# tiantianxuabc/ORB_SLAM2_Refactored

Measured on AMD Instinct MI355X. Metric: frames/sec ORB extract+match (1280×720, 8 lvl, 1000 feat) + LocalBA iters/sec, higher is better.
Workload: dtype u8; 1 GPU; C2: 1280x720 mono, 8 levels, 2000 features, extract + brute-force Hamming top-2/ratio match of every frame vs its predecessor; width=1280, height=720, nlevels=8, nfeatures=2000, parallelism=8192-frame job sharded over 1 GPU(s), 8192 frames per GPU

## Files before the change

orb_slam2_refactored_amd/csrc/orbx.hip:

```cpp
#include <algorithm>
#include <cfloat>
#include <cmath>
#include <cstring>
#include <mutex>
#include <type_traits>
#include <vector>

#include <hip/hip_ext.h>

#include "common.h"
#include "qt_sort.h"
#include "sincos_f.h"
#include "stereo.h"

namespace orbamd {

constexpr int MAX_LEVELS = 16;
constexpr int MAX_ZONE = 64;
constexpr int MAX_ROOTS = 32;
constexpr int PATCH = 43;
constexpr int HBLUR_W = 37;
constexpr int HBS = 40;
static_assert(HBLUR_W + 3 <= HBS, "the blur's fourth-column tiles store up to column 39");

// ... 116 lines not shown
}

template <bool WV>
__device__ __forceinline__ void qt_sync() {
    if constexpr (WV) {
        __builtin_amdgcn_fence(__ATOMIC_ACQ_REL, "workgroup");
        __builtin_amdgcn_wave_barrier();
        asm volatile("s_waitcnt lgkmcnt(0)" ::: "memory");
    } else {
        __syncthreads();
    }
}
template <bool WV>
__device__ __forceinline__ int grp_excl_scan(int v, int* tmp, int* total) {
    if constexpr (WV) {
        const int inc = wave_incl_scan(v);
        *total = __builtin_amdgcn_readlane(inc, 63);
        return inc - v;
    } else {
        return block_excl_scan(v, tmp, total);
    }
}

typedef unsigned short us2 __attribute__((ext_vector_type(2)));

__device__ __forceinline__ uint32_t htap24(uint32_t h) { return h & 0xffff0u; }
__device__ __forceinline__ uint32_t mulhi24(uint32_t a, uint32_t b) {
#ifdef PYR_MULHI_MASK_DIAG
    return __umulhi(a & 0xffffffu, b & 0xffffffu);
#else
    uint32_t r;
    asm("v_mul_hi_u32_u24 %0, %1, %2" : "=v"(r) : "v"(a), "v"(b));
    return r;
#endif
}
__device__ __forceinline__ uint32_t vcoef24(int b) { return ((uint32_t)b & 0xfffu) << 12; }
__device__ __forceinline__ uint32_t vtail(uint32_t h0, uint32_t h1, uint32_t b0_24, uint32_t b1_24) {
    return (__umul24(h0, b0_24 >> 12) + __umul24(h1, b1_24 >> 12) + (1u << 21)) >> 22;
}

__device__ __forceinline__ us2 pyr_tap(uint32_t hi, uint32_t lo, uint32_t sel) {
    const uint32_t r = __builtin_amdgcn_perm(hi, lo, sel);
    return *reinterpret_cast<const us2*>(&r);
}

constexpr int PYR_TW = 64, PYR_TH = 64;
constexpr int PYR_SW = 144, PYR_SH = 128;

__device__ __forceinline__ int4 pyr_row_taps(int2 yv, int sy_lo) {
    return make_int4(((yv.x & 0xffff) - sy_lo) * PYR_SW, ((yv.x >> 16) - sy_lo) * PYR_SW, (int)vcoef24(yv.y),
                     (int)vcoef24(yv.y >> 16));
}

__device__ __forceinline__ void pyr_tile_compute(const Geom& g, const LevelDev& L, int f, uint8_t* pyr,
                                                 const uint8_t* S, const int2* xs_t, const int4* ys_t, int tx0,
                                                 int ty0, int tw, int th, int xa) {
    {
        const int q0 = (threadIdx.x & 15) * 4;
        uint32_t sel0[2], sel1[2];
        int wdb[2];
        us2 a0[2], a1[2];
        bool fits = true;
#pragma unroll
        for (int j = 0; j < 2; j++) {
            const int2 xv0 = xs_t[min(q0 + 2 * j, tw - 1)], xv1 = xs_t[min(q0 + 2 * j + 1, tw - 1)];
            const int s00 = (xv0.x & 0xffff) - xa, s01 = (xv0.x >> 16) - xa;
            const int s10 = (xv1.x & 0xffff) - xa, s11 = (xv1.x >> 16) - xa;
            const int wd = s00 >> 2;
            const int e00 = s00 - 4 * wd, e01 = s01 - 4 * wd, e10 = s10 - 4 * wd, e11 = s11 - 4 * wd;
            fits = fits && max(e01, e11) <= 7 && min(e00, e10) >= 0;
            sel0[j] = (uint32_t)e00 | 0x0c00u | ((uint32_t)e01 << 16) | 0x0c000000u;
            sel1[j] = (uint32_t)e10 | 0x0c00u | ((uint32_t)e11 << 16) | 0x0c000000u;
            wdb[j] = 4 * wd;
            a0[j] = *reinterpret_cast<const us2*>(&xv0.y);
            a1[j] = *reinterpret_cast<const us2*>(&xv1.y);
        }
        if (!__syncthreads_or(!fits)) {
            if (q0 >= tw) return;
            const bool full = q0 + 3 < tw;
            uint8_t* dst = pyr + (long long)f * g.pyr_frame_bytes + L.off + tx0 + q0 +
                           (long long)(ty0 + (int)(threadIdx.x >> 4)) * L.stride;
            const long long dstep = 16ll * L.stride;
            const int tcol = L.tail_x - (tx0 + q0);
            auto rows = [&](auto tail_c) {
                constexpr bool TAIL = decltype(tail_c)::value;
                for (int ty = threadIdx.x >> 4; ty < th; ty += 16, dst += dstep) {
                    const int4 yv = ys_t[ty];
                    const uint32_t b0 = (uint32_t)yv.z, b1 = (uint32_t)yv.w;
                    uint32_t out = 0;
#pragma unroll
                    for (int j = 0; j < 2; j++) {
                        const uint32_t* s0 = reinterpret_cast<const uint32_t*>(S + yv.x + wdb[j]);
                        const uint32_t* s1 = reinterpret_cast<const uint32_t*>(S + yv.y + wdb[j]);
                        const uint32_t w00 = s0[0], w01 = s0[1], w10 = s1[0], w11 = s1[1];
                        const uint32_t r0a = __builtin_amdgcn_udot2(pyr_tap(w01, w00, sel0[j]), a0[j], 0u, false);
                        const uint32_t r1a = __builtin_amdgcn_udot2(pyr_tap(w11, w10, sel0[j]), a0[j], 0u, false);
                        const uint32_t r0b = __builtin_amdgcn_udot2(pyr_tap(w01, w00, sel1[j]), a1[j], 0u, false);
                        const uint32_t r1b = __builtin_amdgcn_udot2(pyr_tap(w11, w10, sel1[j]), a1[j], 0u, false);
                        uint32_t va = (mulhi24(htap24(r0a), b0) + mulhi24(htap24(r1a), b1) + 2) >> 2;
                        uint32_t vb = (mulhi24(htap24(r0b), b0) + mulhi24(htap24(r1b), b1) + 2) >> 2;
                        if (TAIL) {
                            va = 2 * j >= tcol ? vtail(r0a, r1a, b0, b1) : va;
                            vb = 2 * j + 1 >= tcol ? vtail(r0b, r1b, b0, b1) : vb;
                        }
                        out |= (va | (vb << 8)) << (16 * j);
                    }
                    if (full) {
                        *reinterpret_cast<uint32_t*>(dst) = out;
                    } else {
                        for (int k = 0; k < 3; k++)
                            if (q0 + k < tw) dst[k] = (uint8_t)(out >> (8 * k));
                    }
                }
            };
#ifndef PYR_NO_TAIL_DIAG
            if (tx0 + tw > L.tail_x) rows(std::true_type{});
            else
#endif
                rows(std::false_type{});
            return;
        }
    }
    const int q0 = (threadIdx.x & 15) * 4;
    if (q0 >= tw) return;
    uint8_t* dbase = pyr + (long long)f * g.pyr_frame_bytes + L.off + tx0 + q0;
#pragma nounroll
    for (int ty = threadIdx.x >> 4; ty < th; ty += 16) {
        const int4 yv = ys_t[ty];
        const int r0 = yv.x, r1 = yv.y;
        const int b0 = yv.z >> 12, b1 = yv.w >> 12;
        uint32_t packed = 0;
#pragma nounroll
        for (int k = 0; k < 4; k++) {
            const int2 xv = xs_t[min(q0 + k, tw - 1)];
            const int sx0 = (xv.x & 0xffff) - xa, sx1 = (xv.x >> 16) - xa, a0 = xv.y & 0xffff, a1 = xv.y >> 16;
            const int h0 = S[r0 + sx0] * a0 + S[r0 + sx1] * a1;
            const int h1 = S[r1 + sx0] * a0 + S[r1 + sx1] * a1;
            const int s0 = min(h0 >> 4, 32767), s1 = min(h1 >> 4, 32767);
            int v = (((s0 * b0) >> 16) + ((s1 * b1) >> 16) + 2) >> 2;
            if (tx0 + q0 + k >= L.tail_x) v = (h0 * b0 + h1 * b1 + (1 << 21)) >> 22;
            packed |= (uint32_t)(v > 255 ? 255 : v) << (8 * k);
        }
        uint8_t* dst = dbase + (long long)(ty0 + ty) * L.stride;
        if (q0 + 3 < tw) *reinterpret_cast<uint32_t*>(dst) = packed;
        else {
            dst[0] = (uint8_t)packed;
            if (q0 + 1 < tw) dst[1] = (uint8_t)(packed >> 8);
            if (q0 + 2 < tw) dst[2] = (uint8_t)(packed >> 16);
        }
    }
}

constexpr int PYR_PF = 5;

struct PyrTile {
    int f, tx0, ty0, tw, th, sy_lo, xa, nc, items, mul;
    const uint8_t* src;
    int sstep;
};

__device__ __forceinline__ PyrTile pyr_tile_geom(const Geom& g, int l, int t, int ntx, int nty, const uint8_t* in,
                                                 long long in_fstride, int in_step, uint8_t* pyr) {
    const LevelDev& L = g.lv[l];
    const LevelDev& Ls = g.lv[l - 1];
    PyrTile T;
    const int per = ntx * nty;
    T.f = t / per;
    const int r = t - T.f * per;
    T.ty0 = (r / ntx) * PYR_TH;
    T.tx0 = (r - (r / ntx) * ntx) * PYR_TW;
    T.tw = min(PYR_TW, L.w - T.tx0);
    T.th = min(PYR_TH, L.h - T.ty0);
    const int sx_lo = max(0, (int)floor((T.tx0 + 0.5) * L.ssx - 0.5) - 2);
    const int sx_hi = min(Ls.w - 1, (int)floor((T.tx0 + T.tw - 0.5) * L.ssx - 0.5) + 2);
    T.sy_lo = max(0, (int)floor((T.ty0 + 0.5) * L.ssy - 0.5) - 2);
    const int sy_hi = min(Ls.h - 1, (int)floor((T.ty0 + T.th - 0.5) * L.ssy - 0.5) + 2);
    T.xa = sx_lo & ~15;
    T.nc = ((sx_hi - T.xa) >> 4) + 1;
    T.items = (sy_hi - T.sy_lo + 1) * T.nc;
    T.mul = ((1 << 20) + T.nc - 1) / T.nc;
    T.src = level_base(g, l - 1, T.f, in, in_fstride, in_step, pyr, &T.sstep);
    auto u = [](int x) { return __builtin_amdgcn_readfirstlane(x); };
    T.f = u(T.f), T.tx0 = u(T.tx0), T.ty0 = u(T.ty0), T.tw = u(T.tw), T.th = u(T.th), T.sy_lo = u(T.sy_lo);
    T.xa = u(T.xa), T.nc = u(T.nc), T.items = u(T.items), T.mul = u(T.mul), T.sstep = u(T.sstep);
    const unsigned long long sp = (unsigned long long)(uintptr_t)T.src;
    T.src = (const uint8_t*)(uintptr_t)(((unsigned long long)(unsigned)u((int)(sp >> 32)) << 32) |
                                        (unsigned)u((int)(unsigned)sp));
    return T;
}

__device__ __forceinline__ int pyr_piece_row(const PyrTile& T, int i) {
    return (int)(__umulhi(((unsigned)i & 0x7ffu) << 12, (unsigned)T.mul & 0xffffffu) & 0x7ffu);
}
__device__ __forceinline__ int mul12(int a, int b) {
    return (int)(((unsigned)a & 0xfffu) * ((unsigned)b & 0xfffu));
}
__device__ __forceinline__ void pyr_piece_load(const PyrTile& T, int i, uint4& v) {
    if (i < T.items) {
        const int rr = pyr_piece_row(T, i), c = i - mul12(rr, T.nc);
        v = *reinterpret_cast<const uint4*>(T.src + __mul24(T.sy_lo + rr, T.sstep) + T.xa + 16 * c);
    }
}

__device__ __forceinline__ void pyr_fetch(const PyrTile& T, int tid, uint4& v0, uint4& v1, uint4& v2, uint4& v3,
                                          uint4& v4) {
    static_assert(PYR_PF == 5, "five pieces per thread");
    pyr_piece_load(T, tid, v0);
    pyr_piece_load(T, tid + 256, v1);
    pyr_piece_load(T, tid + 512, v2);
    pyr_piece_load(T, tid + 768, v3);
    pyr_piece_load(T, tid + 1024, v4);
}

__device__ __forceinline__ void pyr_stage(const PyrTile& T, int tid, uint8_t* S, const uint4& v, int k) {
    const int i = tid + 256 * k;
    if (i < T.items) {
        const int rr = pyr_piece_row(T, i), c = i - mul12(rr, T.nc);
        *reinterpret_cast<uint4*>(&S[mul12(rr, PYR_SW) + 16 * c]) = v;
    }
}

__global__ __launch_bounds__(256) void pyramid_level_kernel(Geom g, int l, const uint8_t* __restrict__ in,
                                                            long long in_fstride, int in_step, uint8_t* pyr,
                                                            const int2* __restrict__ xtab,
                                                            const int2* __restrict__ ytab) {
    __shared__ __attribute__((aligned(16))) uint8_t S[PYR_SH * PYR_SW + 16];
    __shared__ int2 xs_t[PYR_TW];
    __shared__ int4 ys_t[PYR_TH];
    const LevelDev& L = g.lv[l];
    const LevelDev& Ls = g.lv[l - 1];
    const int gx = gridDim.x, gxy = gridDim.x * gridDim.y;
    const int lb = xcd_swizzle(blockIdx.x + gx * blockIdx.y + gxy * blockIdx.z, gxy * gridDim.z);
    const int f = lb / gxy;
    const int tx0 = (lb % gx) * PYR_TW, ty0 = ((lb % gxy) / gx) * PYR_TH;
    const int tw = min(PYR_TW, L.w - tx0), th = min(PYR_TH, L.h - ty0);
    int sstep;
    const uint8_t* src = level_base(g, l - 1, f, in, in_fstride, in_step, pyr, &sstep);
    const int2* xt = xtab + L.xtab_off;
    const int2* yt = ytab + L.ytab_off;
    const int sw = Ls.w, sh = Ls.h;
    const double scx = L.ssx, scy = L.ssy;
    const int sx_lo = max(0, (int)floor((tx0 + 0.5) * scx - 0.5) - 2);
    const int sx_hi = min(sw - 1, (int)floor((tx0 + tw - 0.5) * scx - 0.5) + 2);
    const int sy_lo = max(0, (int)floor((ty0 + 0.5) * scy - 0.5) - 2);
    if ((int)threadIdx.x < tw) xs_t[threadIdx.x] = xt[tx0 + threadIdx.x];
    if ((int)threadIdx.x >= 64 && (int)threadIdx.x - 64 < th)
        ys_t[threadIdx.x - 64] = pyr_row_taps(yt[ty0 + threadIdx.x - 64], sy_lo);
    const int sy_hi = min(sh - 1, (int)floor((ty0 + th - 0.5) * scy - 0.5) + 2);
    const int xa = sx_lo & ~3;
    const int nd = (sx_hi - xa + 4) >> 2;
    const int nr = sy_hi - sy_lo + 1;
    const bool aligned = ((reinterpret_cast<uintptr_t>(src) | (uintptr_t)sstep) & 3) == 0;
    if (((reinterpret_cast<uintptr_t>(src) | (uintptr_t)sstep) & 15) == 0 && sx_hi - (sx_lo & ~15) < PYR_SW) {
        const PyrTile T = pyr_tile_geom(g, l, lb, gx, gridDim.y, in, in_fstride, in_step, pyr);
        uint4 v0, v1, v2, v3, v4;
        pyr_fetch(T, threadIdx.x, v0, v1, v2, v3, v4);
        pyr_stage(T, threadIdx.x, S, v0, 0);
        pyr_stage(T, threadIdx.x, S, v1, 1);
        pyr_stage(T, threadIdx.x, S, v2, 2);
        pyr_stage(T, threadIdx.x, S, v3, 3);
        pyr_stage(T, threadIdx.x, S, v4, 4);
        __syncthreads();
        pyr_tile_compute(g, L, f, pyr, S, xs_t, ys_t, tx0, ty0, tw, th, T.xa);
        return;
    }
    if (aligned) {
        constexpr int RPW = PYR_SH / 4;
        const int wv = __builtin_amdgcn_readfirstlane((int)(threadIdx.x >> 6));
        const int ln = threadIdx.x & 63;
        const int col = min(xa + 4 * ln, (sw - 1) & ~3);
        const uint8_t* rbase = src + (long long)sy_lo * sstep + col;
        uint32_t v[RPW];
#pragma unroll
        for (int k = 0; k < RPW; k++) {
            const int rk = min(wv + 4 * k, nr - 1);
            v[k] = *reinterpret_cast<const uint32_t*>(rbase + (long long)rk * sstep);
        }
        if (ln < nd) {
            uint32_t* drow = reinterpret_cast<uint32_t*>(S) + wv * (PYR_SW / 4) + ln;
#pragma unroll
            for (int k = 0; k < RPW; k++)
                if (wv + 4 * k < nr) drow[k * PYR_SW] = v[k];
        }
    } else {
        for (int i = threadIdx.x; i < nd * nr; i += blockDim.x) {
            const int r = i / nd, d = i - r * nd;
            const uint8_t* rowp = src + (long long)(sy_lo + r) * sstep;
            const int x = xa + 4 * d;
            uint32_t v = 0;
            for (int q = 0; q < 4; q++)
                if (x + q < sw) v |= (uint32_t)rowp[x + q] << (8 * q);
            *reinterpret_cast<uint32_t*>(&S[r * PYR_SW + 4 * d]) = v;
        }
    }
    __syncthreads();
    pyr_tile_compute(g, L, f, pyr, S, xs_t, ys_t, tx0, ty0, tw, th, xa);
}

constexpr int PP_MAXP = 8;
constexpr int PP_MAXC = 96, PP_MAXR = 96;

__device__ __forceinline__ uint32_t pyr_px_generic(const uint8_t* S, int2 xv, int4 yv, int xa, bool tail) {
    const int r0 = yv.x, r1 = yv.y;
    const int sx0 = (xv.x & 0xffff) - xa, sx1 = (xv.x >> 16) - xa, a0 = xv.y & 0xffff, a1 = xv.y >> 16;
    const int b0 = yv.z >> 12, b1 = yv.w >> 12;
    const int h0 = S[r0 + sx0] * a0 + S[r0 + sx1] * a1;
    const int h1 = S[r1 + sx0] * a0 + S[r1 + sx1] * a1;
    const int s0 = min(h0 >> 4, 32767), s1 = min(h1 >> 4, 32767);
    int v = (((s0 * b0) >> 16) + ((s1 * b1) >> 16) + 2) >> 2;
    if (tail) v = (h0 * b0 + h1 * b1 + (1 << 21)) >> 22;
    return (uint32_t)(v > 255 ? 255 : v);
}

__global__ __launch_bounds__(256) void pyramid_pair_kernel(Geom g, int l, const uint8_t* __restrict__ in,
                                                           long long in_fstride, int in_step, uint8_t* pyr,
                                                           const int2* __restrict__ xtab,
                                                           const int2* __restrict__ ytab) {
    __shared__ __attribute__((aligned(16))) uint8_t S[PYR_SH * PYR_SW + 16];
    __shared__ int2 xs1[PP_MAXC], xs2[PYR_TW];
    __shared__ int4 ys1[PP_MAXR], ys2[PYR_TH];
    const LevelDev& L0 = g.lv[l - 1];
    const LevelDev& L1 = g.lv[l];
    const LevelDev& L2 = g.lv[l + 1];
    const int tid = threadIdx.x;
    const int gx = gridDim.x, gxy = gridDim.x * gridDim.y;
    const int lb = xcd_swizzle(blockIdx.x + gx * blockIdx.y + gxy * blockIdx.z, gxy * gridDim.z);
    const int f = lb / gxy;
    const int tx0 = (lb % gx) * PYR_TW, ty0 = ((lb % gxy) / gx) * PYR_TH;
    const int tw = min(PYR_TW, L2.w - tx0), th = min(PYR_TH, L2.h - ty0);
    auto u = [](int x) { return __builtin_amdgcn_readfirstlane(x); };
    const int ax0 = max(0, (int)floor((tx0 + 0.5) * L2.ssx - 0.5) - 2);
    const int c1 = u(min(L1.w - 1, (int)floor((tx0 + tw - 0.5) * L2.ssx - 0.5) + 2));
    const int ay0 = u(max(0, (int)floor((ty0 + 0.5) * L2.ssy - 0.5) - 2));
    const int ay1 = u(min(L1.h - 1, (int)floor((ty0 + th - 0.5) * L2.ssy - 0.5) + 2));
    const int c0 = u(ax0 & ~3);
    const int ncol = c1 - c0 + 1, nrow = ay1 - ay0 + 1;
    PyrTile T;
    const int bx0 = max(0, (int)floor((c0 + 0.5) * L1.ssx - 0.5) - 2);
    const int bx1 = min(L0.w - 1, (int)floor((c1 + 0.5) * L1.ssx - 0.5) + 2);
    T.sy_lo = u(max(0, (int)floor((ay0 + 0.5) * L1.ssy - 0.5) - 2));
    const int by1 = min(L0.h - 1, (int)floor((ay1 + 0.5) * L1.ssy - 0.5) + 2);
    T.xa = u(bx0 & ~15);
    T.nc = u(((bx1 - T.xa) >> 4) + 1);
    T.items = u((by1 - T.sy_lo + 1) * T.nc);
    T.mul = u(((1 << 20) + T.nc - 1) / T.nc);
    T.src = level_base(g, l - 1, f, in, in_fstride, in_step, pyr, &T.sstep);
    {
        uint4 v0, v1, v2, v3, v4;
        pyr_fetch(T, tid, v0, v1, v2, v3, v4);
        if (tid < ncol) xs1[tid] = xtab[L1.xtab_off + c0 + tid];
// ... 53 lines not shown
                        const uint32_t r0b = __builtin_amdgcn_udot2(pyr_tap(w01, w00, sel1[j]), a1[j], 0u, false);
                        const uint32_t r1b = __builtin_amdgcn_udot2(pyr_tap(w11, w10, sel1[j]), a1[j], 0u, false);
                        uint32_t va = (mulhi24(htap24(r0a), b0) + mulhi24(htap24(r1a), b1) + 2) >> 2;
                        uint32_t vb = (mulhi24(htap24(r0b), b0) + mulhi24(htap24(r1b), b1) + 2) >> 2;
                        if (TAIL) {
                            va = 2 * j >= tcol ? vtail(r0a, r1a, b0, b1) : va;
                            vb = 2 * j + 1 >= tcol ? vtail(r0b, r1b, b0, b1) : vb;
                        }
                        out[pp] |= (va | (vb << 8)) << (16 * j);
                    }
                } else {
#pragma unroll
                    for (int k = 0; k < 4; k++) out[pp] |= pyr_px_generic(S, xv[k], yv, T.xa, k >= tcol) << (8 * k);
                }
            }
        };
#ifndef PYR_NO_TAIL_DIAG
        if (c1 >= L1.tail_x) rows(std::true_type{});
        else
#endif
            rows(std::false_type{});
    }
    __syncthreads();
    if (act) {
        uint8_t* lrow = pyr + (long long)f * g.pyr_frame_bytes + L1.off + c0 + 4 * q;
        const bool full = c0 + 4 * q + 3 <= c1;
#pragma unroll
        for (int pp = 0; pp < PP_MAXP; pp++) {
            const int r = r0 + pp * rpp;
            if (r >= nrow) break;
            *reinterpret_cast<uint32_t*>(&S[r * PYR_SW + 4 * q]) = out[pp];
            uint8_t* dst = lrow + __mul24(ay0 + r, L1.stride);
            if (full) {
                *reinterpret_cast<uint32_t*>(dst) = out[pp];
            } else {
                for (int k = 0; k < 3; k++)
                    if (c0 + 4 * q + k <= c1) dst[k] = (uint8_t)(out[pp] >> (8 * k));
            }
        }
    }
    __syncthreads();
    pyr_tile_compute(g, L2, f, pyr, S, xs2, ys2, tx0, ty0, tw, th, c0);
}

static bool pyr_pair_fits(const Geom& g, int l) {
    const double s1x = g.lv[l].ssx, s1y = g.lv[l].ssy, s2x = g.lv[l + 1].ssx, s2y = g.lv[l + 1].ssy;
    const int ncol = (int)std::ceil(PYR_TW * s2x) + 10, nrow = (int)std::ceil(PYR_TH * s2y) + 7;
    const int ncq = (ncol + 3) / 4, rpp = 256 / ncq;
    const int bw = (int)std::ceil(ncol * s1x) + 7 + 15, bh = (int)std::ceil(nrow * s1y) + 7;
    return ncol + 8 <= PYR_SW && nrow <= PYR_SH && ncol <= PP_MAXC && nrow <= PP_MAXR && (nrow + rpp - 1) / rpp <= PP_MAXP &&
           bw <= PYR_SW && bh <= PYR_SH &&
           bh * ((bw + 15) / 16) <= PYR_PF * 256;
}

typedef _Float16 h8v __attribute__((ext_vector_type(8)));
typedef float pf4v __attribute__((ext_vector_type(4)));
struct PyrMfmaLane { uint32_t a[4]; float c[4]; };
constexpr int PM_MAXB1 = 6;
constexpr int PM_TAB = PYR_SH;
constexpr int PM_MAXU1 = 12;


template <bool TAIL>
__device__ __forceinline__ uint32_t pyr_mfma_unit(const uint8_t* sp, int k, const h8v& A, const pf4v& C, const int4& t,
                                                  int tcol) {
    const int g = lane_id() >> 4;
    constexpr uint32_t hmask = TAIL ? 0xfffffu : 0xffff0u;
    const uint2 w = *reinterpret_cast<const uint2*>(sp + k * (15 * PYR_SW));
    const uint4 bu = make_uint4(__builtin_amdgcn_perm(0x64646464u, w.x, 0x04010400u),
                                __builtin_amdgcn_perm(0x64646464u, w.x, 0x04030402u),
                                __builtin_amdgcn_perm(0x64646464u, w.y, 0x04010400u),
                                __builtin_amdgcn_perm(0x64646464u, w.y, 0x04030402u));
    const pf4v d = __builtin_amdgcn_mfma_f32_16x16x32_f16(A, __builtin_bit_cast(h8v, bu), C, 0, 0, 0);
    const uint32_t b0 = (uint32_t)t.y, b1 = (uint32_t)t.z;
    uint32_t out = 0;
#pragma unroll
    for (int j = 0; j < 4; j++) {
        const uint32_t h0 = __float_as_uint(d[j]) & hmask;
        const uint32_t h1 = (uint32_t)__builtin_amdgcn_mov_dpp((int)h0, 0x101, 0xf, 0xf, true);
        uint32_t v;
        if (!TAIL) {
            v = (mulhi24(h0, b0) + mulhi24(h1, b1) + 2) >> 2;
        } else {
            v = (mulhi24(h0 & 0xffff0u, b0) + mulhi24(h1 & 0xffff0u, b1) + 2) >> 2;
            v = 4 * g + j >= tcol ? vtail(h0, h1, b0, b1) : v;
        }
        out |= v << (8 * j);
    }
    return out;
}

__device__ __forceinline__ void pyr_mfma_frag(const PyrMfmaLane* tab, h8v& A, pf4v& C) {
    const PyrMfmaLane t = tab[lane_id()];
    A = __builtin_bit_cast(h8v, make_uint4(t.a[0], t.a[1], t.a[2], t.a[3]));
    C = pf4v{t.c[0], t.c[1], t.c[2], t.c[3]};
}

__device__ __forceinline__ void pyr_mfma_tab(const int2* ytab, int r0, int nrow, int sy_lo, int ostride, int4* tab) {
    const int y = threadIdx.x;
    if (y < nrow) {
        const int2 v = ytab[r0 + y];
        const int s0 = (v.x & 0xffff) - sy_lo;
        const int s0n = y + 1 < nrow ? (ytab[r0 + y + 1].x & 0xffff) - sy_lo : PM_TAB;
        if (y == 0)
            for (int r = 0; r < s0; r++) tab[r] = make_int4(-1, 0, 0, -1);
        tab[s0] = make_int4((r0 + y) * ostride, (int)vcoef24(v.y), (int)vcoef24(v.y >> 16), y);
// ... 2323 lines not shown
        lbase += q < l ? cq : 0;
        cnt_l = q == l ? cq : cnt_l;
    }
    if (s == 0 && lane == 0) counts[f] = total;
    const int i = s - g.lv[l].out_base;
    if (i >= cnt_l) return;
    const int oidx = lbase + i;
    if (oidx >= cap) return;
#endif
    describe_keypoint<TRIG>(g, l, f, k, (long long)f * cap + oidx, in, in_fstride, in_step, pyr, kps, desc, Hb, lb);
}

__global__ __launch_bounds__(256) void qt_sort_test_kernel(QtItem* items, int n, int* scratch) {
    __shared__ int s_cnt[2];
    qt_sort_block<false>(items, n, scratch, scratch + n, scratch + 2 * n, scratch + 3 * n,
                  reinterpret_cast<QtItem*>(scratch + 4 * n), scratch + 6 * n, n / 3 + 2, s_cnt);
}

}

using namespace orbamd;

struct orbx_extractor {
    orbx_params p;
    int device = 0;
    hipStream_t stream = nullptr;
    std::vector<float> scale, inv_scale, sigma2, inv_sigma2;
    std::vector<int> quota;
    std::mutex mu;

    int g_rows = -1, g_cols = -1;
    Geom geom;
    std::vector<CellDev> cells;
    int NC = 0, PTC = 0;
    size_t qt_lds = 0;
    int qt_ptc0 = 0;
    size_t qt_lds0 = 0;
    int qt_wave = 0, qt_wave_wg = 2, qtw_l0 = 0, qtw_nc = 0, qtw_ptc = 0;
    size_t qtw_lds = 0;
    FastLds fl;
    size_t fast_lds = 0;
    int fast_cpw = 16;
    int fast_spec = 8;
    int fast_pair = 0;
    bool fast_pair_on = false;
    int fast_spec_first = 1;
    int nsub = 1;
    int debug_nc = 0;
    int debug_qt_block = 0;
    uint32_t fault_host = 0;
    int pyr_mfma = 0;
    std::vector<char> pyr_mfma_ok;
    DevBuf d_pyrmt, d_pyrkb;
    int pyr_pair = 2;
    int trig_float = 0;
    int resize_simd = 0;
    std::vector<std::pair<hipStream_t, hipEvent_t>> sub;
    hipEvent_t fork_ev = nullptr;
    bool lvl_overlap = false;
    hipStream_t lvl_side = nullptr;
    hipEvent_t lvl_fork = nullptr, lvl_join = nullptr;
    DevBuf d_cells, d_xtab, d_ytab;
    DevBuf d_strips;
    DevBuf d_slottab;
    DevBuf d_lvlpre;
    std::vector<int> strip_beg;

    int ws_frames = 0;
    DevBuf d_pyr, d_slots, d_cellcnt, d_P, d_T, d_sel, d_selcnt, d_fault;
    DevBuf d_img, d_kps, d_desc, d_counts;
    DevBuf d_stereo_sad;
    int prof = 0;
    std::vector<std::pair<hipEvent_t, hipEvent_t>> prof_ev[4];
    std::vector<hipEvent_t> ev_pool;
    const uint8_t* last_in = nullptr;
    long long last_fstride = 0;
    size_t last_step = 0;
    int last_frames = 0;
    int desc_dense = 0;
    int desc_force_c = 0;
    int desc_c = 0;
    DevBuf d_dstat;
    int32_t* h_dstat = nullptr;
    hipEvent_t dstat_ev = nullptr;
    bool dstat_pending = false;
    bool last_single = false;
    int last_kcap = 0;
    DevBuf d_stereo_out;
    std::vector<uint8_t> h_stage;
};

static int resize_tail_x(int w, int V) {
    if (V <= 0) return w;
    if (V == 1) return 0;
    int x = 0;
    for (; x <= w - V; x += V) {}
    for (; x < w - V / 2; x += V / 2) {}
    return x;
}

static int cv_round_d(double v) { return (int)std::lrint(v); }
static int cv_round_f(float v) { return (int)std::lrintf(v); }

static void compute_tables(orbx_extractor* h) {
    const orbx_params& p = h->p;
    const int L = p.nlevels;
// ... 383 lines not shown
    uint32_t* fault = h->d_fault.as<uint32_t>();
    auto fast = [&](int l0, int l1, hipStream_t s) {
        const int sb = h->strip_beg[l0], ns = h->strip_beg[l1] - sb;
        if (ns <= 0) return;
        const FastLds& fl = h->fl;
        auto kern = h->fast_pair_on ? (fl.CS == 48 && fl.ZS == 36   ? fast_cells_kernel<48, 36, true>
                                       : fl.CS == 52 && fl.ZS == 40 ? fast_cells_kernel<52, 40, true>
                                                                    : fast_cells_kernel<0, 0, true>)
                                    : (fl.CS == 48 && fl.ZS == 36   ? fast_cells_kernel<48, 36, false>
                                       : fl.CS == 52 && fl.ZS == 40 ? fast_cells_kernel<52, 40, false>
                                                                    : fast_cells_kernel<0, 0, false>);
        launch_timed(h, 1, kern, dim3((unsigned)(ns * F)), dim3(64), (uint32_t)h->fast_lds, s,
                           g, h->d_cells.as<CellDev>(), h->d_strips.as<int2>(), d_imgs, fstride, step, pyr, h->p.iniThFAST,
                           h->p.minThFAST, slots, cellcnt, fault, h->fl, sb, ns,
                           h->fast_spec > 0 && h->fast_spec_first ? h->fast_spec | (1 << 29) : h->fast_spec);
    };
    const unsigned qt_block = h->debug_qt_block ? (unsigned)h->debug_qt_block : (unsigned)QT_THREADS;
    auto quadtree = [&](int l0, int nl, hipStream_t s) {
        if (nl <= 0) return;
        const int lw = std::max(l0, h->qtw_l0), nw_lv = l0 + nl - lw;
        if (nw_lv > 0) {
            launch_timed(h, 2, quadtree_kernel<true>, dim3((unsigned)F, (unsigned)((nw_lv + 3) / 4)), dim3(qt_block),
                         (uint32_t)h->qtw_lds, s, g, cellcnt, slots, h->d_cells.as<CellDev>(), Pb, Tb, sel, selcnt, h->qtw_nc,
                         h->qtw_ptc, fault, lw, nw_lv);
            nl -= nw_lv;
            if (nl <= 0) return;
        }
        if (h->qt_ptc0 > 0 && l0 == 0) {
            launch_timed(h, 2, quadtree_kernel<false>, dim3((unsigned)F, 1u), dim3(qt_block), (uint32_t)h->qt_lds0, s, g,
                         cellcnt, slots, h->d_cells.as<CellDev>(), Pb, Tb, sel, selcnt, h->NC, h->qt_ptc0, fault, 0, 1);
            l0 = 1;
            if (--nl <= 0) return;
        }
        launch_timed(h, 2, quadtree_kernel<false>, dim3((unsigned)F, (unsigned)nl), dim3(qt_block), (uint32_t)h->qt_lds, s,
                     g, cellcnt, slots, h->d_cells.as<CellDev>(), Pb, Tb, sel, selcnt, h->NC, h->PTC, fault, l0, nl);
    };
    auto pyramid = [&](int l) -> int {
        const int first = h->pyr_pair == 2 ? 1 : 2;
        const bool a16 = l > 1 || (((uintptr_t)d_imgs | (uintptr_t)fstride | (uintptr_t)step) & 15) == 0;
        if (h->pyr_pair && l >= first && (l - first) % 2 == 0 && l + 1 < g.nlevels && a16 && h->pyr_mfma &&
            h->pyr_mfma_ok[l]) {
            const int ntx = (g.lv[l + 1].w + PYR_TW - 1) / PYR_TW, nty = (g.lv[l + 1].h + PYR_TH - 1) / PYR_TH;
            launch_timed(h, 0, pyramid_pair_mfma_kernel, dim3((unsigned)ntx, (unsigned)nty, (unsigned)F), dim3(256), 0u,
                         st, g, l, d_imgs, fstride, step, pyr, h->d_ytab.as<int2>(), h->d_pyrmt.as<PyrMfmaLane>(),
                         h->d_pyrkb.as<int>());
            return 1;
        }
        if (h->pyr_pair && l >= first && (l - first) % 2 == 0 && l + 1 < g.nlevels && a16 && pyr_pair_fits(g, l)) {
            const int ntx = (g.lv[l + 1].w + PYR_TW - 1) / PYR_TW, nty = (g.lv[l + 1].h + PYR_TH - 1) / PYR_TH;
            launch_timed(h, 0, pyramid_pair_kernel, dim3((unsigned)ntx, (unsigned)nty, (unsigned)F), dim3(256), 0u, st,
                         g, l, d_imgs, fstride, step, pyr, h->d_xtab.as<int2>(), h->d_ytab.as<int2>());
            return 1;
        }
        const int ntx = (g.lv[l].w + PYR_TW - 1) / PYR_TW, nty = (g.lv[l].h + PYR_TH - 1) / PYR_TH;
        launch_timed(h, 0, pyramid_level_kernel, dim3((unsigned)ntx, (unsigned)nty, (unsigned)F), dim3(256), 0u, st, g, l,
                     d_imgs, fstride, step, pyr, h->d_xtab.as<int2>(), h->d_ytab.as<int2>());
        return 0;
    };
    const int nc0 = g.lv[0].ncells;
    if (side && nc0 > 0 && g.nlevels > 1) {
        (void)hipStreamWaitEvent(side, h->lvl_fork, 0);
        fast(0, 1, side);
        quadtree(0, 1, side);
        (void)hipEventRecord(h->lvl_join, side);
        {
            for (int l = 1; l < g.nlevels; l++) l += pyramid(l);
        }
        fast(1, g.nlevels, st);
        quadtree(1, g.nlevels - 1, st);
        (void)hipStreamWaitEvent(st, h->lvl_join, 0);
    } else {
        {
            for (int l = 1; l < g.nlevels; l++) l += pyramid(l);
        }
        fast(0, g.nlevels, st);
        quadtree(0, g.nlevels, st);
    }
    int* lvlpre = h->d_lvlpre.as<int>() + (long long)f0 * LVP;
    if (DESC_SLOT_TAB)
        hipLaunchKernelGGL(describe_prefix_kernel, dim3((unsigned)((F + 255) / 256)), dim3(256), 0, st, (const int*)selcnt,
                           g.nlevels, F, lvlpre, d_counts, h->d_dstat.as<int>());
    const int rows_max = std::min(g.out_frame, cap);
    const int C = (DESC_SLOT_TAB && h->desc_dense) ? std::max(1, std::min(h->desc_c > 0 ? h->desc_c : rows_max, rows_max)) : 0;
    DescGrid dg{};
    if (C > 0) {
        dg.C = C;
        const unsigned d = (unsigned)C;
        int lg = 0;
        while ((1ull << lg) < d) lg++;
        dg.m = (unsigned)((((1ull << lg) - d) << 32) / d + 1);
        dg.s1 = lg > 0 ? 1 : 0;
        dg.s2 = lg > 0 ? lg - 1 : 0;
    }
    launch_timed(h, 3, h->trig_float ? describe_kernel<1> : describe_kernel<0>,
                 dim3((unsigned)(C > 0 ? C : g.out_frame), (unsigned)F), dim3(64), 0u, st, g, d_imgs, fstride, step, pyr,
                 sel, selcnt, d_kps, d_desc, d_counts, cap, h->d_slottab.as<uint32_t>(), lvlpre, dg);
    if (C > 0 && C < rows_max)
        launch_timed(h, 3, h->trig_float ? describe_overflow_kernel<1> : describe_overflow_kernel<0>,
                     dim3((unsigned)std::min(F, 2048)), dim3(64), 0u, st, g, d_imgs, fstride, step, pyr, sel, d_kps, d_desc,
                     cap, (const int*)lvlpre, F, C);
}

static int launch_fast_hint(orbx_extractor* h, hipStream_t st) {
    if (!(h->fast_spec > 0 && h->fast_spec_first)) return ORB_OK;
    const int ns = h->strip_beg[h->geom.nlevels];
    if (ns <= 0) return ORB_OK;
    hipLaunchKernelGGL(fast_hint_kernel, dim3((unsigned)((ns + 255) / 256)), dim3(256), 0, st, h->d_strips.as<int2>(),
                       h->d_cellcnt.as<int>(), ns);
    ORB_HIP_TRY(hipGetLastError());
// ... 67 lines not shown
    }
    ORB_HIP_TRY(hipGetLastError());
    const int rc = describe_grid_end(h, st);
    return rc ? rc : launch_fast_hint(h, st);
}

static int check_fault(orbx_extractor* h) {
    uint32_t f = 0;
    ORB_HIP_TRY(hipMemcpy(&f, h->d_fault.ptr, 4, hipMemcpyDeviceToHost));
    if (f) {
        ORB_HIP_TRY(hipMemset(h->d_fault.ptr, 0, 4));
        set_error("device capacity check failed (fault mask " + std::to_string(f) + ")");
        return ORB_EINTERNAL;
    }
    return ORB_OK;
}

namespace orbamd {
__global__ __launch_bounds__(256) void pack_rows_kernel(const uint4* __restrict__ desc, int cap,
                                                        const int* __restrict__ counts, const int* __restrict__ incl,
                                                        uint4* __restrict__ out, int out_rows) {
    const int f = blockIdx.x;
    const int c = counts[f];
    const int n = min(max(c, 0), cap);
    const long long start = (long long)incl[f] - c;
    const long long r0 = max(start, 0ll), r1 = min(start + n, (long long)out_rows);
    const uint4* src = desc + (long long)f * cap * 2;
    for (long long i = 2 * r0 + threadIdx.x; i < 2 * r1; i += blockDim.x) out[i] = src[i - 2 * start];
}

}

extern "C" {

int orbx_create(const orbx_params* params, int device, orbx_extractor** out) {
    ORB_CHECK_ARG(params && out, "null argument");
    ORB_CHECK_ARG(params->nlevels >= 1 && params->nlevels <= MAX_LEVELS, "nlevels must be in [1,16]");
    ORB_CHECK_ARG(params->nfeatures >= 0 && params->scaleFactor > 1.0f, "bad nfeatures / scaleFactor");
    int ndev = 0;
    ORB_HIP_TRY(hipGetDeviceCount(&ndev));
    ORB_CHECK_ARG(device >= 0 && device < ndev, "no such HIP device");
    ORB_HIP_TRY(hipSetDevice(device));
    orbx_extractor* h = new orbx_extractor();
    h->p = *params;
    h->device = device;
    if (const char* e = getenv("ORBX_FAST_CPW")) h->fast_cpw = std::max(1, std::min(64, atoi(e)));
    if (const char* e = getenv("ORBX_FAST_SPEC")) h->fast_spec = std::max(-1, atoi(e));
    if (const char* e = getenv("ORBX_FAST_PAIR")) h->fast_pair = atoi(e) != 0;
    if (const char* e = getenv("ORBX_QT_WAVE")) h->qt_wave = atoi(e) != 0;
    if (const char* e = getenv("ORBX_QT_WAVE_WG")) h->qt_wave_wg = std::max(1, std::min(4, atoi(e)));
    if (const char* e = getenv("ORBX_FAST_SPEC_FIRST")) h->fast_spec_first = atoi(e) != 0;

    if (const char* e = getenv("ORBX_NSUB")) h->nsub = std::max(1, std::min(8, atoi(e)));
    if (const char* e = getenv("ORBX_PYR_PAIR")) h->pyr_pair = std::max(0, std::min(2, atoi(e)));
    if (const char* e = getenv("ORBX_PYR_MFMA")) h->pyr_mfma = atoi(e) != 0;
    if (const char* e = getenv("ORBX_LEVEL_OVERLAP")) h->lvl_overlap = atoi(e) != 0;
    if (const char* e = getenv("ORBX_DEBUG_NC")) h->debug_nc = atoi(e);
    if (const char* e = getenv("ORBX_DESC_DENSE")) h->desc_dense = atoi(e) != 0;
    if (const char* e = getenv("ORBX_DESC_C")) h->desc_force_c = std::max(0, atoi(e));
    if (const char* e = getenv("ORBX_DEBUG_QT_BLOCK")) {
        const int b = atoi(e);
        if (b >= 64 && b <= QT_THREADS && b % 64 == 0) h->debug_qt_block = b;
    }
    if (const char* e = getenv("ORBX_TRIG")) h->trig_float = (e[0] == 'f' || e[0] == '1') ? 1 : 0;
    if (const char* e = getenv("ORBX_RESIZE_TAIL")) {
        const int v = atoi(e);
        if (v == 0 || v == 1 || v == 8 || v == 16 || v == 32 || v == 64) h->resize_simd = v;
    }
    compute_tables(h);
    hipError_t e = hipStreamCreateWithFlags(&h->stream, hipStreamNonBlocking);
    if (e != hipSuccess) {
        delete h;
        set_error(std::string("hipStreamCreate: ") + hipGetErrorString(e));
        return ORB_EHIP;
    }
    *out = h;
    return ORB_OK;
}

int orbx_destroy(orbx_extractor* h) {
    if (!h) return ORB_OK;
    (void)hipSetDevice(h->device);
    DevBuf* bufs[] = {&h->d_cells, &h->d_strips, &h->d_xtab, &h->d_ytab, &h->d_pyr, &h->d_slots, &h->d_cellcnt, &h->d_P,
                      &h->d_T, &h->d_sel, &h->d_selcnt, &h->d_fault, &h->d_img, &h->d_kps, &h->d_desc,
                      &h->d_counts, &h->d_stereo_sad, &h->d_pyrmt, &h->d_pyrkb, &h->d_slottab, &h->d_lvlpre,
                      &h->d_stereo_out, &h->d_dstat};
    for (DevBuf* b : bufs) b->release();
    for (auto& v : h->prof_ev)
        for (auto& pr : v) { (void)hipEventDestroy(pr.first); (void)hipEventDestroy(pr.second); }
    for (hipEvent_t e : h->ev_pool) (void)hipEventDestroy(e);
    if (h->stream) (void)hipStreamDestroy(h->stream);
    for (auto& se : h->sub) { (void)hipStreamDestroy(se.first); (void)hipEventDestroy(se.second); }
    if (h->fork_ev) (void)hipEventDestroy(h->fork_ev);
    if (h->lvl_side) (void)hipStreamDestroy(h->lvl_side);
    if (h->lvl_fork) (void)hipEventDestroy(h->lvl_fork);
    if (h->lvl_join) (void)hipEventDestroy(h->lvl_join);
    if (h->dstat_ev) (void)hipEventDestroy(h->dstat_ev);
    if (h->h_dstat) (void)hipHostFree(h->h_dstat);
    delete h;
    return ORB_OK;
}

int orbx_set_opencv_compat(orbx_extractor* h, int trig_mode, int resize_simd) {
    ORB_CHECK_ARG(h, "null extractor");
    ORB_CHECK_ARG(trig_mode >= -1 && trig_mode <= 1, "trig_mode must be -1 (keep), 0 (double) or 1 (float)");
    ORB_CHECK_ARG(resize_simd == -1 || resize_simd == 0 || resize_simd == 1 || resize_simd == 8 || resize_simd == 16 ||
// ... 418 lines not shown
```

Before: 174,400 frames/s.

## Reuse horizontal pyramid sums across consecutive rows with taller run-based tiles

Adds a run-based compute path to the pyramid level kernel. Each thread processes five consecutive output rows and reuses the bottom horizontal tap sums as the next row's top when the source row is shared, marked with a 'fresh' flag bit in the row-tap table. Tiles grow from 64 to 80 rows when the staged source fits in shared memory. This is meant to cut redundant horizontal dot products and per-tile overhead, at the cost of a wave-wide ballot per row, an extra masking step in the fallback path, and possible divergence when the fit check fails.

```diff
diff --git a/orb_slam2_refactored_amd/csrc/orbx.hip b/orb_slam2_refactored_amd/csrc/orbx.hip
--- a/orb_slam2_refactored_amd/csrc/orbx.hip
+++ b/orb_slam2_refactored_amd/csrc/orbx.hip
@@ -192,10 +192,127 @@
                      (int)vcoef24(yv.y >> 16));
 }
 
+constexpr int PYR_RUN = 5;
+constexpr int PYR_VTH = 80;
+constexpr int PYR_ROW_FRESH = (int)0x80000000u;
+
+__device__ __forceinline__ int4 pyr_run_taps(const int2* yt, int y0, int i, int lo, int hi, int sy_lo) {
+    const int y = y0 + i;
+    const int2 yv = yt[min(max(y, lo), hi)];
+    int4 t = pyr_row_taps(yv, sy_lo);
+    bool fresh = i % PYR_RUN == 0;
+    if (y >= lo && y <= hi) fresh = fresh || y == lo || (yv.x & 0xffff) != (yt[y - 1].x >> 16);
+    if (fresh) t.w |= PYR_ROW_FRESH;
+    return t;
+}
+
+struct PyrCols {
+    uint32_t sel0[2], sel1[2];
+    int wdb[2];
+    us2 a0[2], a1[2];
+};
+__device__ __forceinline__ bool pyr_cols_setup(PyrCols& C, const int2 (&xv)[4], int xa) {
+    bool fits = true;
+#pragma unroll
+    for (int j = 0; j < 2; j++) {
+        const int2 xv0 = xv[2 * j], xv1 = xv[2 * j + 1];
+        const int s00 = (xv0.x & 0xffff) - xa, s01 = (xv0.x >> 16) - xa;
+        const int s10 = (xv1.x & 0xffff) - xa, s11 = (xv1.x >> 16) - xa;
+        const int wd = s00 >> 2;
+        const int e00 = s00 - 4 * wd, e01 = s01 - 4 * wd, e10 = s10 - 4 * wd, e11 = s11 - 4 * wd;
+        fits = fits && max(e01, e11) <= 7 && min(e00, e10) >= 0;
+        C.sel0[j] = (uint32_t)e00 | 0x0c00u | ((uint32_t)e01 << 16) | 0x0c000000u;
+        C.sel1[j] = (uint32_t)e10 | 0x0c00u | ((uint32_t)e11 << 16) | 0x0c000000u;
+        C.wdb[j] = 4 * wd;
+        C.a0[j] = *reinterpret_cast<const us2*>(&xv0.y);
+        C.a1[j] = *reinterpret_cast<const us2*>(&xv1.y);
+    }
+    return fits;
+}
+struct PyrH { uint32_t a[2], b[2]; };
+template <bool TAIL>
+__device__ __forceinline__ void pyr_hsums(PyrH& h, const uint8_t* S, int off, const PyrCols& C) {
+#pragma unroll
+    for (int j = 0; j < 2; j++) {
+        const uint32_t* s = reinterpret_cast<const uint32_t*>(S + off + C.wdb[j]);
+        const uint32_t w0 = s[0], w1 = s[1];
+        const uint32_t ra = __builtin_amdgcn_udot2(pyr_tap(w1, w0, C.sel0[j]), C.a0[j], 0u, false);
+        const uint32_t rb = __builtin_amdgcn_udot2(pyr_tap(w1, w0, C.sel1[j]), C.a1[j], 0u, false);
+        h.a[j] = TAIL ? ra : htap24(ra);
+        h.b[j] = TAIL ? rb : htap24(rb);
+    }
+}
+template <bool TAIL>
+__device__ __forceinline__ uint32_t pyr_vrow(const PyrH& h0, const PyrH& h1, uint32_t b0, uint32_t b1, int tcol) {
+    uint32_t out = 0;
+#pragma unroll
+    for (int j = 0; j < 2; j++) {
+        uint32_t va, vb;
+        if (!TAIL) {
+            va = (mulhi24(h0.a[j], b0) + mulhi24(h1.a[j], b1) + 2) >> 2;
+            vb = (mulhi24(h0.b[j], b0) + mulhi24(h1.b[j], b1) + 2) >> 2;
+        } else {
+            const uint32_t c0 = b0 & 0xffffffu, c1 = b1 & 0xffffffu;
+            va = (mulhi24(htap24(h0.a[j]), c0) + mulhi24(htap24(h1.a[j]), c1) + 2) >> 2;
+            vb = (mulhi24(htap24(h0.b[j]), c0) + mulhi24(htap24(h1.b[j]), c1) + 2) >> 2;
+            va = 2 * j >= tcol ? vtail(h0.a[j], h1.a[j], c0, c1) : va;
+            vb = 2 * j + 1 >= tcol ? vtail(h0.b[j], h1.b[j], c0, c1) : vb;
+        }
+        out |= (va | (vb << 8)) << (16 * j);
+    }
+    return out;
+}
+template <bool TAIL, class Put>
+__device__ __forceinline__ void pyr_run_rows(const uint8_t* S, const int4* yr, const PyrCols& C, int tcol, Put put) {
+    PyrH top, bot;
+#pragma unroll
+    for (int k = 0; k < PYR_RUN; k++) {
+        const int4 yv = yr[k];
+        if (k == 0 || __builtin_amdgcn_ballot_w64(yv.w < 0) != 0) pyr_hsums<TAIL>(top, S, yv.x, C);
+        else top = bot;
+        pyr_hsums<TAIL>(bot, S, yv.y, C);
+        put(k, pyr_vrow<TAIL>(top, bot, (uint32_t)yv.z, (uint32_t)yv.w, tcol));
+    }
+}
+
+__device__ __forceinline__ bool pyr_tile_compute_runs(const Geom& g, const LevelDev& L, int f, uint8_t* pyr,
+                                                      const uint8_t* S, const int2* xs_t, const int4* ys_t, int tx0,
+                                                      int ty0, int tw, int th, int xa) {
+    const int q0 = (threadIdx.x & 15) * 4;
+    PyrCols C;
+    int2 xv[4];
+#pragma unroll
+    for (int k = 0; k < 4; k++) xv[k] = xs_t[min(q0 + k, tw - 1)];
+    const bool fits = pyr_cols_setup(C, xv, xa);
+    if (__syncthreads_or(!fits)) return false;
+    const int r0 = PYR_RUN * (int)(threadIdx.x >> 4);
+    if (q0 >= tw || r0 >= th) return true;
+    const bool full = q0 + 3 < tw;
+    uint8_t* dst = pyr + (long long)f * g.pyr_frame_bytes + L.off + tx0 + q0 + (long long)(ty0 + r0) * L.stride;
+    const int tcol = L.tail_x - (tx0 + q0);
+    auto put = [&](int k, uint32_t out) {
+        if (r0 + k < th) {
+            uint8_t* d = dst + (long long)k * L.stride;
+            if (full) {
+                *reinterpret_cast<uint32_t*>(d) = out;
+            } else {
+                for (int c = 0; c < 3; c++)
+                    if (q0 + c < tw) d[c] = (uint8_t)(out >> (8 * c));
+            }
+        }
+    };
+    if (tx0 + tw > L.tail_x) pyr_run_rows<true>(S, ys_t + r0, C, tcol, put);
+    else pyr_run_rows<false>(S, ys_t + r0, C, tcol, put);
+    return true;
+}
+
+template <bool RUN = false>
 __device__ __forceinline__ void pyr_tile_compute(const Geom& g, const LevelDev& L, int f, uint8_t* pyr,
                                                  const uint8_t* S, const int2* xs_t, const int4* ys_t, int tx0,
                                                  int ty0, int tw, int th, int xa) {
-    {
+    if constexpr (RUN) {
+        if (pyr_tile_compute_runs(g, L, f, pyr, S, xs_t, ys_t, tx0, ty0, tw, th, xa)) return;
+    } else {
         const int q0 = (threadIdx.x & 15) * 4;
         uint32_t sel0[2], sel1[2];
         int wdb[2];
@@ -268,7 +385,7 @@
     for (int ty = threadIdx.x >> 4; ty < th; ty += 16) {
         const int4 yv = ys_t[ty];
         const int r0 = yv.x, r1 = yv.y;
-        const int b0 = yv.z >> 12, b1 = yv.w >> 12;
+        const int b0 = yv.z >> 12, b1 = (yv.w >> 12) & 0xfff;
         uint32_t packed = 0;
 #pragma nounroll
         for (int k = 0; k < 4; k++) {
@@ -299,6 +416,7 @@
     int sstep;
 };
 
+template <int TH>
 __device__ __forceinline__ PyrTile pyr_tile_geom(const Geom& g, int l, int t, int ntx, int nty, const uint8_t* in,
                                                  long long in_fstride, int in_step, uint8_t* pyr) {
     const LevelDev& L = g.lv[l];
@@ -307,10 +425,10 @@
     const int per = ntx * nty;
     T.f = t / per;
     const int r = t - T.f * per;
-    T.ty0 = (r / ntx) * PYR_TH;
+    T.ty0 = (r / ntx) * TH;
     T.tx0 = (r - (r / ntx) * ntx) * PYR_TW;
     T.tw = min(PYR_TW, L.w - T.tx0);
-    T.th = min(PYR_TH, L.h - T.ty0);
+    T.th = min(TH, L.h - T.ty0);
     const int sx_lo = max(0, (int)floor((T.tx0 + 0.5) * L.ssx - 0.5) - 2);
     const int sx_hi = min(Ls.w - 1, (int)floor((T.tx0 + T.tw - 0.5) * L.ssx - 0.5) + 2);
     T.sy_lo = max(0, (int)floor((T.ty0 + 0.5) * L.ssy - 0.5) - 2);
@@ -360,20 +478,21 @@
     }
 }
 
-__global__ __launch_bounds__(256) void pyramid_level_kernel(Geom g, int l, const uint8_t* __restrict__ in,
-                                                            long long in_fstride, int in_step, uint8_t* pyr,
-                                                            const int2* __restrict__ xtab,
-                                                            const int2* __restrict__ ytab) {
+template <int TH>
+__device__ __forceinline__ void pyramid_level_body(const Geom& g, int l, const uint8_t* __restrict__ in,
+                                                   long long in_fstride, int in_step, uint8_t* pyr,
+                                                   const int2* __restrict__ xtab, const int2* __restrict__ ytab) {
+    constexpr bool RUN = TH == PYR_VTH;
     __shared__ __attribute__((aligned(16))) uint8_t S[PYR_SH * PYR_SW + 16];
     __shared__ int2 xs_t[PYR_TW];
-    __shared__ int4 ys_t[PYR_TH];
+    __shared__ int4 ys_t[TH];
     const LevelDev& L = g.lv[l];
     const LevelDev& Ls = g.lv[l - 1];
     const int gx = gridDim.x, gxy = gridDim.x * gridDim.y;
     const int lb = xcd_swizzle(blockIdx.x + gx * blockIdx.y + gxy * blockIdx.z, gxy * gridDim.z);
     const int f = lb / gxy;
-    const int tx0 = (lb % gx) * PYR_TW, ty0 = ((lb % gxy) / gx) * PYR_TH;
-    const int tw = min(PYR_TW, L.w - tx0), th = min(PYR_TH, L.h - ty0);
+    const int tx0 = (lb % gx) * PYR_TW, ty0 = ((lb % gxy) / gx) * TH;
+    const int tw = min(PYR_TW, L.w - tx0), th = min(TH, L.h - ty0);
     int sstep;
     const uint8_t* src = level_base(g, l - 1, f, in, in_fstride, in_step, pyr, &sstep);
     const int2* xt = xtab + L.xtab_off;
@@ -384,15 +503,20 @@
     const int sx_hi = min(sw - 1, (int)floor((tx0 + tw - 0.5) * scx - 0.5) + 2);
     const int sy_lo = max(0, (int)floor((ty0 + 0.5) * scy - 0.5) - 2);
     if ((int)threadIdx.x < tw) xs_t[threadIdx.x] = xt[tx0 + threadIdx.x];
-    if ((int)threadIdx.x >= 64 && (int)threadIdx.x - 64 < th)
-        ys_t[threadIdx.x - 64] = pyr_row_taps(yt[ty0 + threadIdx.x - 64], sy_lo);
+    if constexpr (RUN) {
+        if ((int)threadIdx.x >= 64 && (int)threadIdx.x - 64 < TH)
+            ys_t[threadIdx.x - 64] = pyr_run_taps(yt, ty0, (int)threadIdx.x - 64, ty0, ty0 + th - 1, sy_lo);
+    } else {
+        if ((int)threadIdx.x >= 64 && (int)threadIdx.x - 64 < th)
+            ys_t[threadIdx.x - 64] = pyr_row_taps(yt[ty0 + threadIdx.x - 64], sy_lo);
+    }
     const int sy_hi = min(sh - 1, (int)floor((ty0 + th - 0.5) * scy - 0.5) + 2);
     const int xa = sx_lo & ~3;
     const int nd = (sx_hi - xa + 4) >> 2;
     const int nr = sy_hi - sy_lo + 1;
     const bool aligned = ((reinterpret_cast<uintptr_t>(src) | (uintptr_t)sstep) & 3) == 0;
     if (((reinterpret_cast<uintptr_t>(src) | (uintptr_t)sstep) & 15) == 0 && sx_hi - (sx_lo & ~15) < PYR_SW) {
-        const PyrTile T = pyr_tile_geom(g, l, lb, gx, gridDim.y, in, in_fstride, in_step, pyr);
+        const PyrTile T = pyr_tile_geom<TH>(g, l, lb, gx, gridDim.y, in, in_fstride, in_step, pyr);
         uint4 v0, v1, v2, v3, v4;
         pyr_fetch(T, threadIdx.x, v0, v1, v2, v3, v4);
         pyr_stage(T, threadIdx.x, S, v0, 0);
@@ -401,7 +525,7 @@
         pyr_stage(T, threadIdx.x, S, v3, 3);
         pyr_stage(T, threadIdx.x, S, v4, 4);
         __syncthreads();
-        pyr_tile_compute(g, L, f, pyr, S, xs_t, ys_t, tx0, ty0, tw, th, T.xa);
+        pyr_tile_compute<RUN>(g, L, f, pyr, S, xs_t, ys_t, tx0, ty0, tw, th, T.xa);
         return;
     }
     if (aligned) {
@@ -434,8 +558,17 @@
         }
     }
     __syncthreads();
-    pyr_tile_compute(g, L, f, pyr, S, xs_t, ys_t, tx0, ty0, tw, th, xa);
-}
+    pyr_tile_compute<RUN>(g, L, f, pyr, S, xs_t, ys_t, tx0, ty0, tw, th, xa);
+}
+
+#define PYR_KERNEL(name, body, th)                                                                              \
+    __global__ __launch_bounds__(256) void name(Geom g, int l, const uint8_t* __restrict__ in, long long in_fstride, \
+                                                int in_step, uint8_t* pyr, const int2* __restrict__ xtab,           \
+                                                const int2* __restrict__ ytab) {                                    \
+        body<th>(g, l, in, in_fstride, in_step, pyr, xtab, ytab);                                                   \
+    }
+PYR_KERNEL(pyramid_level_kernel, pyramid_level_body, PYR_VTH)
+PYR_KERNEL(pyramid_level64_kernel, pyramid_level_body, PYR_TH)
 
 constexpr int PP_MAXP = 8;
 constexpr int PP_MAXC = 96, PP_MAXR = 96;
@@ -595,6 +728,8 @@
            bw <= PYR_SW && bh <= PYR_SH &&
            bh * ((bw + 15) / 16) <= PYR_PF * 256;
 }
+
+static bool pyr_level_run_fits(const Geom& g, int l) { return g.lv[l].ssy * PYR_VTH + 6 <= PYR_SH; }
 
 typedef _Float16 h8v __attribute__((ext_vector_type(8)));
 typedef float pf4v __attribute__((ext_vector_type(4)));
@@ -3024,6 +3159,7 @@
     int pyr_mfma = 0;
     std::vector<char> pyr_mfma_ok;
     DevBuf d_pyrmt, d_pyrkb;
+    int pyr_run = 1;
     int pyr_pair = 2;
     int trig_float = 0;
     int resize_simd = 0;
@@ -3513,9 +3649,12 @@
                          g, l, d_imgs, fstride, step, pyr, h->d_xtab.as<int2>(), h->d_ytab.as<int2>());
             return 1;
         }
-        const int ntx = (g.lv[l].w + PYR_TW - 1) / PYR_TW, nty = (g.lv[l].h + PYR_TH - 1) / PYR_TH;
-        launch_timed(h, 0, pyramid_level_kernel, dim3((unsigned)ntx, (unsigned)nty, (unsigned)F), dim3(256), 0u, st, g, l,
-                     d_imgs, fstride, step, pyr, h->d_xtab.as<int2>(), h->d_ytab.as<int2>());
+        const bool run = h->pyr_run && pyr_level_run_fits(g, l);
+        const int tile_h = run ? PYR_VTH : PYR_TH;
+        const int ntx = (g.lv[l].w + PYR_TW - 1) / PYR_TW, nty = (g.lv[l].h + tile_h - 1) / tile_h;
+        launch_timed(h, 0, run ? pyramid_level_kernel : pyramid_level64_kernel,
+                     dim3((unsigned)ntx, (unsigned)nty, (unsigned)F), dim3(256), 0u, st, g, l, d_imgs, fstride, step, pyr,
+                     h->d_xtab.as<int2>(), h->d_ytab.as<int2>());
         return 0;
     };
     const int nc0 = g.lv[0].ncells;
@@ -3689,6 +3828,7 @@
     if (const char* e = getenv("ORBX_FAST_SPEC_FIRST")) h->fast_spec_first = atoi(e) != 0;
 
     if (const char* e = getenv("ORBX_NSUB")) h->nsub = std::max(1, std::min(8, atoi(e)));
+    if (const char* e = getenv("ORBX_PYR_RUN")) h->pyr_run = atoi(e) != 0;
     if (const char* e = getenv("ORBX_PYR_PAIR")) h->pyr_pair = std::max(0, std::min(2, atoi(e)));
     if (const char* e = getenv("ORBX_PYR_MFMA")) h->pyr_mfma = atoi(e) != 0;
     if (const char* e = getenv("ORBX_LEVEL_OVERLAP")) h->lvl_overlap = atoi(e) != 0;
```

Result: no change. 174,300 frames/s (-0.0%).
